# jwliao1209/DiffMusic

Hardware: AMD Instinct MI355X
Metric: denoising steps/sec (10 s clip, 200-step DPS) (higher is better)
Workload: dtype f16; 1 GPU; MusicLDM + DPS music_inpainting, 10 s @16 kHz, 200-step schedule, batch 8 per GPU (BASELINE.json configs[1]); global_batch=8, clips_per_gpu=8, lanes=1, parallelism=clip-sharded x1 (RCCL world size 1, no per-step collective), finite=True, nan_steps=0, settle_steps=10, cached_reference_transform=True, launched_by=single process

## Files before the change

diffmusic_amd/_lib.py:

```python
import ctypes as C
import os

_HERE = os.path.dirname(os.path.abspath(__file__))
LIB_PATH = os.environ.get("DMX_LIB_PATH") or os.path.join(_HERE, "lib", "libdiffmusic_hip.so")
MAX_STAGES = 8


class HifiGanConfig(C.Structure):
    _fields_ = [("model_in_dim", C.c_int), ("upsample_initial_channel", C.c_int), ("num_upsamples", C.c_int),
                ("upsample_rates", C.c_int * MAX_STAGES), ("upsample_kernel_sizes", C.c_int * MAX_STAGES),
                ("num_kernels", C.c_int), ("resblock_kernel_sizes", C.c_int * MAX_STAGES),
                ("num_dilations", C.c_int), ("resblock_dilation_sizes", C.c_int * (MAX_STAGES * MAX_STAGES)),
                ("leaky_relu_slope", C.c_float)]


class VaeConfig(C.Structure):
    _fields_ = [("latent_channels", C.c_int), ("out_channels", C.c_int), ("num_blocks", C.c_int),
                ("block_out_channels", C.c_int * MAX_STAGES), ("layers_per_block", C.c_int),
                ("norm_num_groups", C.c_int), ("eps", C.c_float)]


class UNetConfig(C.Structure):
    _fields_ = [("in_channels", C.c_int), ("out_channels", C.c_int), ("num_blocks", C.c_int),
                ("block_out_channels", C.c_int * MAX_STAGES), ("layers_per_block", C.c_int),
# ... 46 lines not shown
    "dmx_model_param_numel": (C.c_size_t, [C.c_void_p, C.c_int]),
    "dmx_model_param_ndim": (C.c_int, [C.c_void_p, C.c_int]),
    "dmx_model_param_dim": (C.c_int, [C.c_void_p, C.c_int, C.c_int]),
    "dmx_model_load_param": (C.c_int, [C.c_void_p, C.c_char_p, C.c_void_p, C.c_size_t]),
    "dmx_model_finalize": (C.c_int, [C.c_void_p, C.c_void_p]),
    "dmx_hifigan_out_len": (C.c_int, [C.c_void_p, C.c_int]),
    "dmx_hifigan_workspace_bytes": (C.c_size_t, [C.c_void_p, C.c_int, C.c_int]),
    "dmx_hifigan_fwd": (C.c_int, [C.c_void_p, C.c_void_p, C.c_void_p, C.c_int, C.c_int, C.c_void_p, C.c_size_t, C.c_void_p]),
    "dmx_hifigan_bwd": (C.c_int, [C.c_void_p, C.c_void_p, C.c_void_p, C.c_void_p]),
    "dmx_hifigan_fwd_dead": (C.c_int, [C.c_void_p, C.c_void_p, C.c_void_p, C.c_int, C.c_int, C.c_int, C.c_int, C.c_void_p, C.c_size_t,
                                       C.c_void_p]),
    "dmx_hifigan_dead_plan": (C.c_int, [C.c_void_p, C.POINTER(C.c_int), C.POINTER(C.c_int), C.POINTER(C.c_int), C.POINTER(C.c_int), C.c_int]),
    "dmx_conv_dead_rows": (C.c_int, [C.c_int] * 9 + [C.POINTER(C.c_int), C.POINTER(C.c_int)]),
    "dmx_vae_workspace_bytes": (C.c_size_t, [C.c_void_p, C.c_int, C.c_int, C.c_int]),
    "dmx_vae_decode_fwd": (C.c_int, [C.c_void_p, C.c_void_p, C.c_float, C.c_void_p, C.c_void_p, C.c_int, C.c_int, C.c_int,
                                     C.c_int, C.c_void_p, C.c_size_t, C.c_void_p]),
    "dmx_vae_decode_bwd": (C.c_int, [C.c_void_p, C.c_void_p, C.c_float, C.c_void_p, C.c_void_p]),
    "dmx_vae_encoder_create": (C.c_void_p, [C.POINTER(VaeConfig)]),
    "dmx_vae_encoder_workspace_bytes": (C.c_size_t, [C.c_void_p, C.c_int, C.c_int, C.c_int]),
    "dmx_vae_encode_fwd": (C.c_int, [C.c_void_p, C.c_void_p, C.c_float, C.c_void_p, C.c_int, C.c_int, C.c_int, C.c_void_p, C.c_size_t,
                                     C.c_void_p]),
    "dmx_latent_init": (C.c_int, [C.c_void_p] * 6 + [C.c_int] * 3 + [C.c_float] * 3 + [C.c_void_p]),
    "dmx_conv2d_raw": (C.c_int, [C.c_void_p] * 4 + [C.c_int] * 9 + [C.c_void_p]),
    "dmx_unet_workspace_bytes": (C.c_size_t, [C.c_void_p, C.c_int, C.c_int, C.c_int]),
    "dmx_unet_fwd": (C.c_int, [C.c_void_p, C.c_void_p, C.c_void_p, C.c_void_p, C.c_void_p, C.c_int, C.c_int, C.c_int,
                               C.c_void_p, C.c_size_t, C.c_void_p]),
    "dmx_unet_fwd_ctx": (C.c_int, [C.c_void_p] * 5 + [C.c_int, C.c_void_p, C.c_int, C.c_void_p, C.c_void_p, C.c_int, C.c_int, C.c_int,
                                   C.c_void_p, C.c_size_t, C.c_void_p]),
    "dmx_unet_workspace_bytes_ctx": (C.c_size_t, [C.c_void_p, C.c_int, C.c_int, C.c_int, C.c_int, C.c_int]),
    "dmx_htsat_create": (C.c_void_p, [C.POINTER(HtsatConfig)]),
    "dmx_htsat_feature_dims": (C.c_int, [C.c_void_p, C.POINTER(C.c_int), C.POINTER(C.c_int)]),
    "dmx_htsat_workspace_bytes": (C.c_size_t, [C.c_void_p, C.c_int, C.c_int]),
    "dmx_htsat_fwd": (C.c_int, [C.c_void_p, C.c_void_p, C.c_int, C.c_int, C.c_void_p, C.c_int, C.c_void_p, C.c_size_t, C.c_void_p]),
    "dmx_htsat_bwd": (C.c_int, [C.c_void_p, C.c_void_p, C.c_void_p, C.c_void_p, C.c_void_p]),
    "dmx_htsat_tape_raw": (C.c_size_t, [C.c_void_p, C.c_int, C.c_int, C.c_int, C.c_void_p, C.c_size_t, C.c_void_p]),
    "dmx_htsat_ln_rows_fwd_raw": (C.c_int, [C.c_void_p] * 4 + [C.c_longlong] + [C.c_int] * 4 + [C.c_float, C.c_int, C.c_void_p]),
    "dmx_htsat_ln_rows_bwd_raw": (C.c_int, [C.c_void_p] * 5 + [C.c_longlong] + [C.c_int] * 4 + [C.c_float, C.c_int, C.c_void_p]),
    "dmx_htsat_gelu_fwd_raw": (C.c_int, [C.c_void_p, C.c_void_p, C.c_longlong, C.c_void_p]),
    "dmx_htsat_gelu_bwd_raw": (C.c_int, [C.c_void_p, C.c_void_p, C.c_void_p, C.c_longlong, C.c_void_p]),
    "dmx_htsat_win_attn_fwd_raw": (C.c_int, [C.c_void_p] * 3 + [C.c_int] * 6 + [C.c_void_p]),
    "dmx_htsat_win_attn_bwd_raw": (C.c_int, [C.c_void_p] * 4 + [C.c_int] * 6 + [C.c_void_p]),
    "dmx_htsat_embed_fwd_raw": (C.c_int, [C.c_void_p, C.c_void_p, C.c_int, C.c_int, C.c_void_p, C.c_void_p]),
    "dmx_htsat_embed_bwd_raw": (C.c_int, [C.c_void_p, C.c_void_p, C.c_int, C.c_int] + [C.c_void_p] * 5),
    "dmx_gram_fwd": (C.c_int, [C.c_void_p, C.c_void_p, C.c_int, C.c_int, C.c_int, C.c_void_p]),
    "dmx_gram_bwd": (C.c_int, [C.c_void_p, C.c_void_p, C.c_void_p, C.c_int, C.c_int, C.c_int, C.c_void_p]),
    "dmx_gemm_raw": (C.c_int, [C.c_void_p, C.c_size_t, C.c_void_p]),
# ... 167 lines not shown
```

diffmusic_amd/csrc/capi.hip:

```cpp
#include "conv_pair.h"
#include "models.h"

#define M_IMPL(m) ((m) ? (m)->impl : nullptr)
#define ST(s) ((hipStream_t)(s))

extern "C" {

int dmx_abi_version(void) { return DMX_ABI_VERSION; }
int dmx_act_dtype(void) { return DMX_ACT_DTYPE; }

dmx_model* dmx_hifigan_create(const dmx_hifigan_config* cfg) {
  if (!cfg || cfg->num_upsamples > DMX_MAX_STAGES || cfg->num_kernels > DMX_MAX_STAGES || cfg->num_dilations > DMX_MAX_STAGES) {
    dmx_set_error("bad hifigan config");
    return nullptr;
  }
  return new dmx_model{dmx_make_hifigan(cfg)};
}
dmx_model* dmx_vae_decoder_create(const dmx_vae_config* cfg) {
  if (!cfg || cfg->num_blocks > DMX_MAX_STAGES) { dmx_set_error("bad vae config"); return nullptr; }
  Model* m = dmx_make_vae(cfg);
  return m ? new dmx_model{m} : nullptr;
}
dmx_model* dmx_unet_create(const dmx_unet_config* cfg) {
  if (!cfg || cfg->num_blocks > DMX_MAX_STAGES) { dmx_set_error("bad unet config"); return nullptr; }
// ... 74 lines not shown
dmx_model* dmx_vae_encoder_create(const dmx_vae_config* cfg) {
  if (!cfg || cfg->num_blocks > DMX_MAX_STAGES) { dmx_set_error("bad vae config"); return nullptr; }
  Model* m = dmx_make_vae_encoder(cfg);
  return m ? new dmx_model{m} : nullptr;
}
size_t dmx_vae_encoder_workspace_bytes(dmx_model* m, int batch, int frames, int bins) {
  if (!m || !m->impl || m->impl->kind != DMX_MODEL_VAE_ENC) return 0;
  return dmx_vae_enc_ws_impl(m->impl, batch, frames, bins);
}
int dmx_vae_encode_fwd(dmx_model* m, const float* mel, float log_floor, float* moments, int batch, int frames, int bins, void* ws,
                       size_t ws_bytes, void* stream) {
  int rc = check(m, DMX_MODEL_VAE_ENC);
  if (rc) return rc;
  if (!ws) { dmx_set_error("null workspace"); return DMX_ERR_WORKSPACE; }
  return dmx_vae_enc_fwd_impl(m->impl, mel, log_floor, moments, batch, frames, bins, ws, ws_bytes, ST(stream));
}
int dmx_latent_init(const float* moments, float* mean, float* logvar, float* x, const float* eps, const float* noise, int batch,
                    int latent_channels, int hw, float sqrt_abar, float scaling_factor, float sqrt_1m_abar, void* stream) {
  return dmx_latent_init_impl(moments, mean, logvar, x, eps, noise, batch, latent_channels, hw, sqrt_abar, scaling_factor, sqrt_1m_abar, ST(stream));
}
int dmx_conv2d_raw(const float* w_host, const float* b_host, const void* x, void* y, int B, int Hi, int Wi, int Ci, int Co, int k, int stride,
                   int pad_lo, int pad_hi, void* stream) {
  return dmx_conv2d_raw_impl(w_host, b_host, (const act_t*)x, (act_t*)y, B, Hi, Wi, Ci, Co, k, stride, pad_lo, pad_hi, ST(stream));
}

dmx_model* dmx_htsat_create(const dmx_htsat_config* cfg) {
  Model* impl = dmx_make_htsat(cfg);
  if (!impl) return nullptr;
  return new dmx_model{impl};
}
int dmx_htsat_feature_dims(dmx_model* m, int* tokens, int* channels) {
  if (!m || !m->impl || m->impl->kind != DMX_MODEL_HTSAT) { dmx_set_error("wrong model handle"); return DMX_ERR_STATE; }
  dmx_htsat_dims_impl(m->impl, tokens, channels);
  return DMX_OK;
}
size_t dmx_htsat_workspace_bytes(dmx_model* m, int batch, int frames) {
  if (!m || !m->impl || m->impl->kind != DMX_MODEL_HTSAT) return 0;
  return dmx_htsat_ws_impl(m->impl, batch, frames);
}
int dmx_htsat_fwd(dmx_model* m, const float* mel, int batch, int frames, float* feat, int keep_state, void* ws, size_t ws_bytes, void* stream) {
  int rc = check(m, DMX_MODEL_HTSAT);
  if (rc) return rc;
  if (!ws) { dmx_set_error("null workspace"); return DMX_ERR_WORKSPACE; }
  return dmx_htsat_fwd_impl(m->impl, mel, batch, frames, feat, keep_state, ws, ws_bytes, ST(stream));
}
int dmx_htsat_bwd(dmx_model* m, const float* dfeat, const float* scale, float* dmel, void* stream) {
// ... 259 lines not shown
```

diffmusic_amd/csrc/kernels.h:

```cpp
#pragma once
#include "dmx_common.h"

#define DMX_GN_MAX_CHUNKS 512

size_t dmx_gn_scratch_floats(int B, int C, int G);
struct GnRegion {
  float* part = nullptr;
  int tm = 0, P = 0, nq = 0;
  int qoff = 0, cq = 0;
};
struct GnParts { int n = 0; GnRegion r[8]; };
size_t dmx_gn_part_floats(int B, int P, int N);
int dmx_groupnorm_fwd(const act_t* x, act_t* y, const float* gamma, const float* beta, float* stats, float* scale,
                      float* shift, float* partial, int B, int P, int C, int G, float eps, int silu, hipStream_t st,
                      const GnParts* parts = nullptr);
int dmx_groupnorm_bwd(const act_t* x, const act_t* dy, const act_t* add, act_t* dx, const float* stats,
                      const float* scale, const float* shift, float* k0, float* k1, float* partial, int B, int P, int C,
                      int G, int silu, hipStream_t st, const GnParts* parts = nullptr);
int dmx_layernorm_fwd(const act_t* x, act_t* y, const float* gamma, const float* beta, int rows, int C, float eps,
                      hipStream_t st);
int dmx_softmax_fwd(const float* S, act_t* P, const float* colbias, long long rows, int N, long long lds, long long ldp,
                    int rows_per_bias, hipStream_t st);
int dmx_softmax_act(const act_t* S, act_t* P, const float* colbias, long long rows, int N, long long ldp, int rows_per_bias,
                    hipStream_t st);
// ... 5 lines not shown
int dmx_transpose(const act_t* in, act_t* out, int R, int C, long long ldi, long long ldo, int Z, int Zi, long long sIo,
                  long long sIi, long long sOo, long long sOi, hipStream_t st);
int dmx_concat2(const act_t* a, const act_t* b, act_t* dst, long long rows, int Ca, int Cb, hipStream_t st);
int dmx_copy_channels(const act_t* src, act_t* dst, long long rows, int C, int lds, int ldd, int soff, int doff,
                      hipStream_t st);
int dmx_axpby(const act_t* x, const act_t* y0, act_t* y, float a, float b, long long n, hipStream_t st);
int dmx_nchw_f32_to_nhwc_bf16(const float* x, act_t* y, int B, int C, int HW, int Cp, float scale, hipStream_t st);
int dmx_nhwc_bf16_to_nchw_f32(const act_t* x, float* y, int B, int C, int HW, int Cp, float scale, hipStream_t st);
int dmx_f32_to_bf16(const float* x, act_t* y, long long n, float scale, hipStream_t st);
int dmx_bf16_to_f32(const act_t* x, float* y, long long n, float scale, hipStream_t st);
int dmx_extract_col(const act_t* x, float* y, long long rows, int ld, int col, hipStream_t st);
int dmx_gather_col_f32(const float* x, float* y, long long rows, int ld, int col, hipStream_t st);
int dmx_tanh_bwd_pad8(const float* dwav, const float* wav8, act_t* gz, long long rows, hipStream_t st);
int dmx_gather_col_f32_dead(const float* x, float* y, long long rows, int ld, int col, int T, int s0, int s1, hipStream_t st);
int dmx_tanh_bwd_pad8_dead(const float* dwav, const float* wav8, act_t* gz, long long rows, int T, int s0, int s1, hipStream_t st);
int dmx_scatter_col_pad8(const float* v, act_t* y, long long rows, float scale, hipStream_t st);
int dmx_gather_col_f32_to_act(const float* x, act_t* y, long long rows, int ld, int col, hipStream_t st);
int dmx_pad_col8_act(const act_t* v, act_t* y, long long rows, hipStream_t st);
int dmx_timestep_embed(const float* t, act_t* y, int B, int dim, hipStream_t st);

bool dmx_flash_attn_ok(int dh, int C);
int dmx_flash_attn_fwd(const act_t* q, const act_t* k, const act_t* v, act_t* o, const float* colbias, int B, int Nq, int Nk,
                       int C, int heads, float scale, hipStream_t st, int ldq = 0, int ldk = 0, int ldv = 0, int* qt_out = nullptr);

int dmx_stft_tables(float* table, float* tableT, int n_fft, int bins, int Npad, int Kpad, int hann, hipStream_t st);
int dmx_stft_fwd(const float* wav, long long wav_stride, const float* table, float* X, int B, int L, int T, int n_fft, int hop, int Npad,
                 hipStream_t st);
int dmx_stft_bwd_frames(const float* Y, const float* tableT, float* dframe, int M, int n_fft, int Kpad, hipStream_t st);
int dmx_mel_fwd(const float* X, const float* fb, float* mel_lin, float* mel_out, int rows, int ldx, int bins, int n_mels, int power2,
                int to_db, float lo, float hi, hipStream_t st);
int dmx_mel_bwd(const float* X, const float* fb, const float* mel_lin, const float* dmel, float* Y, int rows, int ldx, int ldy, int bins,
                int n_mels, int power2, int to_db, float lo, float hi, hipStream_t st);
int dmx_stft_mag(const float* X, float* mag, int B, int T, int bins, int ldx, hipStream_t st);
int dmx_stft_mag_bwd(const float* X, const float* dmag, float* Y, int B, int T, int bins, int ldx, int ldy, hipStream_t st);
int dmx_overlap_add(const float* dframe, float* dwav, long long out_stride, int B, int T, int L, int n_fft, int hop, int accumulate,
                    hipStream_t st);
int dmx_l2_loss_grad(const float* ref, const float* pred, float* loss, float* dpred, int B, long long n, long long ref_stride, float gscale,
                     hipStream_t st);
int dmx_mask_mul(const float* x, long long xs, const float* mask, float* y, long long ys, int B, int L, int Ly, hipStream_t st);
int dmx_melscale(const float* mag, const float* fb, float* mel, int B, int T, int bins, int n_mels, float lo, float hi, hipStream_t st);
int dmx_absmax_normalize(float* x, float* inv_scale, int B, long long n, float target, hipStream_t st);

struct DmxStftMelTables {
  const float2* tw;
  const float* win;
  const int *klo, *klen; const float* fbc; int kmax;
// ... 40 lines not shown
```

diffmusic_amd/csrc/layers.h:

```cpp
#pragma once
#include <string>
#include <vector>
#include <map>
#include <cstdio>
#include <cstring>
#include "dmx_common.h"
#include "kernels.h"

void dmx_set_error(const char* fmt, ...);

inline int pad8(int c) { return (c + 7) & ~7; }

struct Arena {
  char* base = nullptr;
  size_t cap = 0, off = 0, peak = 0;
  bool overflow = false;
  void reset(void* b, size_t c) { base = (char*)b; cap = c; off = 0; overflow = false; }
  void* raw(size_t bytes) {
    bytes = align_up(bytes, 256);
    if (off + bytes > cap) { overflow = true; off += bytes; if (off > peak) peak = off; return base; }
    void* p = base + off;
    off += bytes;
    if (off > peak) peak = off;
    return p;
// ... 72 lines not shown
ConvLayer make_linear(ParamStore& ps, const std::string& prefix, int Ci, int Co, bool bias, bool need_bwd);
int pack_layer(ParamStore& ps, ConvLayer& L, hipStream_t st);
int pack_linear_stack(ParamStore& ps, ConvLayer& dst, const ConvLayer* const* src, int n, hipStream_t st);

int conv_out_len(const ConvLayer& L, int Ti);
int conv_fwd_1d(const ConvLayer& L, const act_t* in, void* out, int B, int Ti, const Epi& e, hipStream_t st);
int conv_bwd_1d(const ConvLayer& L, const act_t* dout, void* din, int B, int Ti, const Epi& e, hipStream_t st);
int conv_fwd_1d_desc(const ConvLayer& L, const act_t* in, void* out, int B, int Ti, const Epi& e, GemmDesc& d);
int conv_bwd_1d_desc(const ConvLayer& L, const act_t* dout, void* din, int B, int Ti, const Epi& e, GemmDesc& d);
struct PairDead;
int conv_pair_run(const GemmDesc& a, const GemmDesc& b, hipStream_t st, const PairDead* dead = nullptr);
int conv_fwd_2d(const ConvLayer& L, const act_t* in, void* out, int B, int Hi, int Wi, const Epi& e, hipStream_t st, int* gn_rows = nullptr);
int pack_layer_up2x(ParamStore& ps, ConvLayer& L, hipStream_t st);
int conv_up2x_fwd(const ConvLayer& L, const act_t* in, void* out, int B, int Hi, int Wi, const Epi& e, hipStream_t st,
                  float* const* gn_buf = nullptr, int* gn_rows = nullptr);
int conv_up2x_bwd(const ConvLayer& L, const act_t* dout, void* din, int B, int Hi, int Wi, const Epi& e, hipStream_t st);
int conv_bwd_2d(const ConvLayer& L, const act_t* dout, void* din, int B, int Hi, int Wi, const Epi& e, hipStream_t st, int* gn_rows = nullptr);
struct GemmBatch { int Z = 1, Zi = 1; long long sAo = 0, sAi = 0, sBo = 0, sBi = 0, sCo = 0, sCi = 0; };
int gemm_nt(const act_t* A, int lda, const act_t* Bm, int ldb, void* C, int ldc, int M, int N, int K, const Epi& e,
            const GemmBatch& gb, hipStream_t st);
int linear_fwd(const ConvLayer& L, const act_t* in, int lda, void* out, int ldc, long long rows, const Epi& e, hipStream_t st);
int linear_bwd(const ConvLayer& L, const act_t* dout, int lda, void* din, int ldc, long long rows, const Epi& e, hipStream_t st);

struct GroupNormLayer {
  int C = 0, G = 32, g_id = -1, b_id = -1;
  float eps = 1e-5f;
};
GroupNormLayer make_gn(ParamStore& ps, const std::string& prefix, int C, int G, float eps);
struct GnSave { float* stats = nullptr; float* scale = nullptr; float* shift = nullptr; };
```

diffmusic_amd/csrc/layers.hip:

```cpp
#include "layers.h"
#include "conv_pair.h"
#include <cstdarg>

static thread_local char g_err[512] = "";
void dmx_set_error(const char* fmt, ...) {
  va_list ap;
  va_start(ap, fmt);
  vsnprintf(g_err, sizeof(g_err), fmt, ap);
  va_end(ap);
}
extern "C" const char* dmx_last_error() { return g_err; }

int ParamStore::add(const std::string& name, std::vector<int> shape) {
  Param p;
  p.name = name;
  p.shape = shape;
  p.numel = 1;
  for (int s : shape) p.numel *= (size_t)s;
  p.dev = (float*)dalloc(p.numel * sizeof(float));
  index[name] = (int)params.size();
  params.push_back(p);
  return (int)params.size() - 1;
}
void* ParamStore::dalloc(size_t bytes) {
// ... 275 lines not shown
  return rc;
}

static void init_desc(GemmDesc& d, const Epi& e) {
  memset(&d, 0, sizeof(d));
  d.Z = 1; d.Zi = 1;
  d.sy = d.sx = 1; d.osy = d.osx = 1;
  d.alpha = e.alpha; d.act_slope = e.act_slope; d.mask_slope = e.mask_slope; d.resid_inv_slope = e.resid_inv_slope;
  d.flags = e.flags;
  d.R = e.R; d.X = e.X; d.C2 = e.C2; d.rowbias = e.rowbias; d.ldrb = e.ldrb;
  d.XB = e.XB; d.B2 = e.B2;
  d.rowstats_out = e.rowstats_out; d.rowstats_in = e.rowstats_in; d.nslots = e.nslots;
  d.gn_part = e.gn_part;
  if (e.gn_part) d.flags |= e.gnb_x ? EPI_GNBWD : EPI_GNSTATS;
  d.gnb_x = e.gnb_x; d.gnb_scale = e.gnb_scale; d.gnb_shift = e.gnb_shift; d.gnb_silu = e.gnb_silu;
  d.gnb_stats = e.gnb_stats; d.gnb_cpg = e.gnb_cpg;
}
static void set_out(GemmDesc& d, void* C, int Ho, int Wo, int ldc) {
  d.C = C; d.Ho = Ho; d.Wo = Wo; d.ldc = d.ldr = d.ldx = d.ldc2 = ldc;
  d.ldxb = d.ldb2 = ldc >> 3;
  d.gnb_ldx = ldc;
}

int conv_out_len(const ConvLayer& L, int Ti) {
  if (L.transposed) return (Ti - 1) * L.stride - 2 * L.pad_w + L.kw;
  return (Ti + 2 * L.pad_w - L.dil * (L.kw - 1) - 1) / L.stride + 1;
}

static void fwd_1d_common(GemmDesc& d, const ConvLayer& L, const act_t* in, void* out, int Ti, int To, const Epi& e) {
  init_desc(d, e);
  if (L.has_bias) { d.bias = L.bias; d.flags |= EPI_BIAS; }
  d.A = in; d.Hi = 1; d.Wi = Ti; d.Ci = L.Cip; d.lda = L.Cip;
  d.N = L.Cop;
  set_out(d, out, 1, To, L.Cop);
}
int conv_fwd_1d_desc(const ConvLayer& L, const act_t* in, void* out, int B, int Ti, const Epi& e, GemmDesc& d) {
  if (L.transposed) return DMX_ERR_SHAPE;
  const int To = conv_out_len(L, Ti);
  fwd_1d_common(d, L, in, out, Ti, To, e);
  d.W = L.wf[0]; d.ntaps = L.kw; d.K = L.kw * L.Cip; d.ldw = d.K;
  d.Hq = 1; d.Wq = To; d.sx = L.stride; d.M = B * To;
  for (int t = 0; t < L.kw; ++t) { d.tdy[t] = 0; d.tdx[t] = (signed char)(t * L.dil - L.pad_w); }
  return DMX_OK;
}

int conv_fwd_1d(const ConvLayer& L, const act_t* in, void* out, int B, int Ti, const Epi& e, hipStream_t st) {
  const int To = conv_out_len(L, Ti);
  GemmDesc d;
  if (!L.transposed) {
    const int rc = conv_fwd_1d_desc(L, in, out, B, Ti, e, d);
    return rc != DMX_OK ? rc : dmx_gemm_launch(d, st);
  }
  fwd_1d_common(d, L, in, out, Ti, To, e);
  const int s = L.stride, p = L.pad_w;
  for (int r = 0; r < s; ++r) {
    GemmDesc q = d;
    const int nt = (int)L.wf_taps[r].size();
    const int base = (r + p) / s;
    q.W = L.wf[r]; q.ntaps = nt; q.K = nt * L.Cip; q.ldw = q.K;
    q.Hq = 1; q.Wq = cdiv(To - r, s); q.M = B * q.Wq;
    q.osx = s; q.oox = r;
    for (int i = 0; i < nt; ++i) { q.tdy[i] = 0; q.tdx[i] = (signed char)(base - i); }
    if (q.Wq <= 0) continue;
    const int rc = dmx_gemm_launch(q, st);
    if (rc != DMX_OK) return rc;
  }
  return DMX_OK;
}

int conv_bwd_1d_desc(const ConvLayer& L, const act_t* dout, void* din, int B, int Ti, const Epi& e, GemmDesc& d) {
  if (!L.wb) { dmx_set_error("layer has no dgrad weights"); return DMX_ERR_STATE; }
  const int To = conv_out_len(L, Ti);
  init_desc(d, e);
  d.A = dout; d.Hi = 1; d.Wi = To; d.Ci = L.Cop; d.lda = L.Cop;
  d.W = L.wb; d.ntaps = L.kw; d.K = L.kw * L.Cop; d.ldw = d.K;
  d.N = L.Cip;
  d.Hq = 1; d.Wq = Ti; d.M = B * Ti;
  set_out(d, din, 1, Ti, L.Cip);
  if (!L.transposed) {
    if (L.stride != 1) return DMX_ERR_SHAPE;
    for (int t = 0; t < L.kw; ++t) { d.tdy[t] = 0; d.tdx[t] = (signed char)(L.pad_w - t * L.dil); }
  } else {
    d.sx = L.stride;
    for (int t = 0; t < L.kw; ++t) { d.tdy[t] = 0; d.tdx[t] = (signed char)(t - L.pad_w); }
  }
  return DMX_OK;
}
int conv_bwd_1d(const ConvLayer& L, const act_t* dout, void* din, int B, int Ti, const Epi& e, hipStream_t st) {
  GemmDesc d;
  const int rc = conv_bwd_1d_desc(L, dout, din, B, Ti, e, d);
  return rc != DMX_OK ? rc : dmx_gemm_launch(d, st);
}

int conv_pair_run(const GemmDesc& a, const GemmDesc& b, hipStream_t st, const PairDead* dead) {
  if (dmx_conv_pair_eligible(&a, b)) return dmx_conv_pair_launch(&a, b, st, dead);
  if (dead) { dmx_set_error("conv_pair_run: dead rows need the fused pair kernel"); return DMX_ERR_SHAPE; }
  const int rc = dmx_gemm_launch(a, st);
  return rc != DMX_OK ? rc : dmx_gemm_launch(b, st);
}

int conv_fwd_2d(const ConvLayer& L, const act_t* in, void* out, int B, int Hi, int Wi, const Epi& e, hipStream_t st, int* gn_rows) {
  const int Ho = (Hi + L.pad_h + L.pad_h_hi - L.kh) / L.stride + 1, Wo = (Wi + L.pad_w + L.pad_w_hi - L.kw) / L.stride + 1;
  GemmDesc d;
  init_desc(d, e);
  if (L.has_bias) { d.bias = L.bias; d.flags |= EPI_BIAS; }
  d.A = in; d.Hi = Hi; d.Wi = Wi; d.Ci = L.Cip; d.lda = L.Cip;
  d.W = L.wf[0]; d.ntaps = L.kh * L.kw; d.K = d.ntaps * L.Cip; d.ldw = d.K;
  d.N = L.Cop; d.Hq = Ho; d.Wq = Wo; d.sy = d.sx = L.stride; d.M = B * Ho * Wo;
  set_out(d, out, Ho, Wo, L.Cop);
  for (int ky = 0; ky < L.kh; ++ky)
    for (int kx = 0; kx < L.kw; ++kx) {
      d.tdy[ky * L.kw + kx] = (signed char)(ky - L.pad_h);
      d.tdx[ky * L.kw + kx] = (signed char)(kx - L.pad_w);
    }
  return dmx_gemm_launch(d, st, gn_rows);
}

int conv_up2x_fwd(const ConvLayer& L, const act_t* in, void* out, int B, int Hi, int Wi, const Epi& e, hipStream_t st,
                  float* const* gn_buf, int* gn_rows) {
  if (L.wup.size() != 4) { dmx_set_error("layer has no upsample-folded weights"); return DMX_ERR_STATE; }
  for (int py = 0; py < 2; ++py)
    for (int px = 0; px < 2; ++px) {
      GemmDesc d;
      Epi ep = e;
      if (gn_buf) ep.gn_part = gn_buf[py * 2 + px];
      init_desc(d, ep);
      if (L.has_bias) { d.bias = L.bias; d.flags |= EPI_BIAS; }
      d.A = in; d.Hi = Hi; d.Wi = Wi; d.Ci = L.Cip; d.lda = L.Cip;
      d.W = L.wup[py * 2 + px]; d.ntaps = 4; d.K = 4 * L.Cip; d.ldw = d.K;
      d.N = L.Cop; d.Hq = Hi; d.Wq = Wi; d.M = B * Hi * Wi;
      set_out(d, out, 2 * Hi, 2 * Wi, L.Cop);
      d.osy = d.osx = 2; d.ooy = py; d.oox = px;
      for (int ty = 0; ty < 2; ++ty)
        for (int tx = 0; tx < 2; ++tx) {
          d.tdy[ty * 2 + tx] = (signed char)up2x_delta(py, ty);
          d.tdx[ty * 2 + tx] = (signed char)up2x_delta(px, tx);
        }
// ... 16 lines not shown
      const int t = (py * 2 + ty) * 4 + (px * 2 + tx);
      d.tdy[t] = (signed char)(py - 2 * up2x_delta(py, ty));
      d.tdx[t] = (signed char)(px - 2 * up2x_delta(px, tx));
    }
  return dmx_gemm_launch(d, st);
}

int conv_bwd_2d(const ConvLayer& L, const act_t* dout, void* din, int B, int Hi, int Wi, const Epi& e, hipStream_t st, int* gn_rows) {
  if (!L.wb) { dmx_set_error("layer has no dgrad weights"); return DMX_ERR_STATE; }
  if (L.stride != 1) return DMX_ERR_SHAPE;
  if (L.pad_h_hi != L.pad_h || L.pad_w_hi != L.pad_w) { dmx_set_error("conv dgrad of an asymmetrically padded layer is not built"); return DMX_ERR_SHAPE; }
  const int Ho = Hi + 2 * L.pad_h - L.kh + 1, Wo = Wi + 2 * L.pad_w - L.kw + 1;
  GemmDesc d;
  init_desc(d, e);
  d.A = dout; d.Hi = Ho; d.Wi = Wo; d.Ci = L.Cop; d.lda = L.Cop;
  d.W = L.wb; d.ntaps = L.kh * L.kw; d.K = d.ntaps * L.Cop; d.ldw = d.K;
  d.N = L.Cip; d.Hq = Hi; d.Wq = Wi; d.M = B * Hi * Wi;
  set_out(d, din, Hi, Wi, L.Cip);
  for (int ky = 0; ky < L.kh; ++ky)
    for (int kx = 0; kx < L.kw; ++kx) {
      d.tdy[ky * L.kw + kx] = (signed char)(L.pad_h - ky);
      d.tdx[ky * L.kw + kx] = (signed char)(L.pad_w - kx);
    }
  return dmx_gemm_launch(d, st, gn_rows);
}

int gemm_nt(const act_t* A, int lda, const act_t* Bm, int ldb, void* C, int ldc, int M, int N, int K, const Epi& e,
            const GemmBatch& gb, hipStream_t st) {
  GemmDesc d;
  init_desc(d, e);
  d.A = A; d.Hi = 1; d.Wi = M; d.Ci = K; d.lda = lda;
  d.W = Bm; d.ntaps = 1; d.K = K; d.ldw = ldb;
  d.N = N; d.Hq = 1; d.Wq = M; d.M = M;
  set_out(d, C, 1, M, ldc);
  d.Z = gb.Z; d.Zi = gb.Zi;
  d.sAo = gb.sAo; d.sAi = gb.sAi; d.sWo = gb.sBo; d.sWi = gb.sBi; d.sCo = gb.sCo; d.sCi = gb.sCi;
  return dmx_gemm_launch(d, st);
}

int linear_fwd(const ConvLayer& L, const act_t* in, int lda, void* out, int ldc, long long rows, const Epi& e, hipStream_t st) {
  Epi ee = e;
  GemmDesc d;
  init_desc(d, ee);
  if (L.has_bias) { d.bias = L.bias; d.flags |= EPI_BIAS; }
  d.A = in; d.Hi = 1; d.Wi = (int)rows; d.Ci = L.Cip; d.lda = lda;
  d.W = L.wf[0]; d.ntaps = 1; d.K = L.Cip; d.ldw = L.Cip;
  d.N = L.Cop; d.Hq = 1; d.Wq = (int)rows; d.M = (int)rows;
  set_out(d, out, 1, (int)rows, ldc);
  if (L.geglu) d.flags |= EPI_GEGLU;
  if (L.colsum) {
    if (!e.rowstats_in || e.nslots * 32 != L.Cip) { dmx_set_error("LayerNorm-folded layer needs the row statistics of its input"); return DMX_ERR_STATE; }
    d.flags |= EPI_LNFOLD; d.colsum = L.colsum; d.ln_eps = L.ln_eps;
    d.flags &= ~EPI_BIAS;
  }
  return dmx_gemm_launch(d, st);
}
int linear_bwd(const ConvLayer& L, const act_t* dout, int lda, void* din, int ldc, long long rows, const Epi& e, hipStream_t st) {
  if (!L.wb) { dmx_set_error("layer has no dgrad weights"); return DMX_ERR_STATE; }
  GemmDesc d;
  init_desc(d, e);
  d.A = dout; d.Hi = 1; d.Wi = (int)rows; d.Ci = L.Cop; d.lda = lda;
  d.W = L.wb; d.ntaps = 1; d.K = L.Cop; d.ldw = L.Cop;
  d.N = L.Cip; d.Hq = 1; d.Wq = (int)rows; d.M = (int)rows;
  set_out(d, din, 1, (int)rows, ldc);
  return dmx_gemm_launch(d, st);
}
```

include/diffmusic_hip.h:

```cpp
#ifndef DIFFMUSIC_HIP_H
#define DIFFMUSIC_HIP_H
#include <stddef.h>
#include <stdint.h>

#ifdef __cplusplus
extern "C" {
#endif

#define DMX_ABI_VERSION 4
#define DMX_MAX_STAGES 8

typedef struct dmx_model dmx_model;

typedef struct dmx_hifigan_config {
  int model_in_dim;
  int upsample_initial_channel;
  int num_upsamples;
  int upsample_rates[DMX_MAX_STAGES];
  int upsample_kernel_sizes[DMX_MAX_STAGES];
  int num_kernels;
  int resblock_kernel_sizes[DMX_MAX_STAGES];
  int num_dilations;
  int resblock_dilation_sizes[DMX_MAX_STAGES * DMX_MAX_STAGES];
  float leaky_relu_slope;
// ... 226 lines not shown
                          int ldk, int ldv, int C, int heads, float scale, int* qt_out, void* stream);
int dmx_softmax_raw(const float* S, void* P, const float* colbias, long long rows, int N, long long lds, long long ldp, int rows_per_bias,
                    void* stream);
int dmx_softmax_act_raw(const void* S, void* P, const float* colbias, long long rows, int N, long long ldp, int rows_per_bias, void* stream);
int dmx_transpose_raw(const void* in, void* out, int R, int C, long long ldi, long long ldo, int Z, int Zi, long long sIo, long long sIi,
                      long long sOo, long long sOi, void* stream);
int dmx_rowdot_raw(const void* a, const void* b, float* out, long long rows, int C, long long lda, long long ldb, void* stream);
int dmx_layernorm_raw(const void* x, void* y, const float* gamma, const float* beta, int rows, int C, float eps, void* stream);
int dmx_geglu_raw(const void* x, void* y, long long rows, int I, void* stream);
int dmx_gemm_splitk_workspace(void* ws, size_t bytes);
int dmx_conv_pair_raw(const void* desc_a, const void* desc_b, size_t desc_bytes, void* stream);
int dmx_conv_pair_dead_raw(const void* desc_a, const void* desc_b, size_t desc_bytes, const int* dead, int* skipped, int* total, void* stream);
int dmx_conv_pair_group_raw(int n, const void* descs_a, const void* descs_b, size_t desc_bytes, void* stream);
int dmx_conv_pair_group_dead_raw(int n, const void* descs_a, const void* descs_b, size_t desc_bytes, const int* dead, void* stream);
size_t dmx_groupnorm_scratch_floats(int B, int C, int G);
int dmx_groupnorm_raw(const void* x, void* y, const float* gamma, const float* beta, float* stats, float* scale, float* shift,
                      float* partial, int B, int P, int C, int G, float eps, int silu, void* stream);
size_t dmx_groupnorm_part_floats(int B, int P, int N);
int dmx_groupnorm_parts_raw(const void* x, void* y, const float* gamma, const float* beta, float* stats, float* scale, float* shift,
                            int B, int P, int C, int G, float eps, int silu, int nreg, float* const* part, const int* geom, void* stream);
int dmx_gemm_last_tile_rows_raw(void);
int dmx_conv2d_raw(const float* w_host, const float* b_host, const void* x, void* y, int B, int Hi, int Wi, int Ci, int Co, int k, int stride,
                   int pad_lo, int pad_hi, void* stream);
int dmx_groupnorm_bwd_raw(const void* x, const void* dy, const void* add, void* dx, const float* stats, const float* scale, const float* shift,
                          float* k0, float* k1, float* partial, int B, int P, int C, int G, int silu, int nreg, float* const* part,
                          const int* geom, void* stream);
int dmx_htsat_ln_rows_fwd_raw(const void* x, void* y, const float* gamma, const float* beta, long long rows, int C, int merge, int H, int W,
                              float eps, int out_fp32, void* stream);
int dmx_htsat_ln_rows_bwd_raw(const void* x, const void* dy, const void* add, void* dx, const float* gamma, long long rows, int C, int merge,
                              int H, int W, float eps, int dy_fp32, void* stream);
int dmx_htsat_gelu_fwd_raw(const void* u, void* y, long long n8, void* stream);
int dmx_htsat_gelu_bwd_raw(const void* u, const void* dy, void* du, long long n8, void* stream);
int dmx_htsat_win_attn_fwd_raw(const void* qkv, void* out, const float* bias_table, int B, int H, int W, int C, int heads, int shift,
                               void* stream);
int dmx_htsat_win_attn_bwd_raw(const void* qkv, const void* dout, void* dqkv, const float* bias_table, int B, int H, int W, int C, int heads,
                               int shift, void* stream);
int dmx_htsat_embed_fwd_raw(dmx_model* m, const float* mel, int batch, int frames, void* tokens, void* stream);
int dmx_htsat_embed_bwd_raw(dmx_model* m, const float* mel, int batch, int frames, const void* dtok, const float* scale, float* dimg,
                            float* dmel, void* stream);

#ifdef __cplusplus
}
#endif
#endif
```

Baseline: 27.47 steps/s (weak scaling: one step advances a batch of 8 clips on one GPU; value = K / wall x 1 GPU(s)).

## Add narrow-output conv kernels for head convolutions with few output channels

Adds dedicated HIP kernels for convolutions whose output is at most 8 channels (padded to 8), such as the HiFi-GAN output conv and VAE conv_out. The forward kernel stages an input halo slab in LDS and uses packed fdot2 dot products, with optional split-K reduction. A separate dgrad kernel handles the single-output 1D backward with the mask epilogue. These replace the general GEMM path, whose tiles are mostly wasted when N is 8. It also adds a test hook for the new path and a DMX_NO_NARROW env switch. The risk is extra code paths with their own edge cases, including numerics that differ from the GEMM path.

Result: no change. 27.56 steps/s (weak scaling: one step advances a batch of 8 clips on one GPU; value = K / wall x 1 GPU(s)) (median of 6 runs) (+0.3%).

```diff
diff --git a/diffmusic_amd/_lib.py b/diffmusic_amd/_lib.py
--- a/diffmusic_amd/_lib.py
+++ b/diffmusic_amd/_lib.py
@@ -92,6 +92,7 @@
                                      C.c_void_p]),
     "dmx_latent_init": (C.c_int, [C.c_void_p] * 6 + [C.c_int] * 3 + [C.c_float] * 3 + [C.c_void_p]),
     "dmx_conv2d_raw": (C.c_int, [C.c_void_p] * 4 + [C.c_int] * 9 + [C.c_void_p]),
+    "dmx_head_conv_raw": (C.c_int, [C.c_int] + [C.c_void_p] * 5 + [C.c_int] * 7 + [C.c_float, C.c_float, C.POINTER(C.c_int), C.c_void_p]),
     "dmx_unet_workspace_bytes": (C.c_size_t, [C.c_void_p, C.c_int, C.c_int, C.c_int]),
     "dmx_unet_fwd": (C.c_int, [C.c_void_p, C.c_void_p, C.c_void_p, C.c_void_p, C.c_void_p, C.c_int, C.c_int, C.c_int,
                                C.c_void_p, C.c_size_t, C.c_void_p]),
diff --git a/diffmusic_amd/csrc/capi.hip b/diffmusic_amd/csrc/capi.hip
--- a/diffmusic_amd/csrc/capi.hip
+++ b/diffmusic_amd/csrc/capi.hip
@@ -120,6 +120,12 @@
 int dmx_conv2d_raw(const float* w_host, const float* b_host, const void* x, void* y, int B, int Hi, int Wi, int Ci, int Co, int k, int stride,
                    int pad_lo, int pad_hi, void* stream) {
   return dmx_conv2d_raw_impl(w_host, b_host, (const act_t*)x, (act_t*)y, B, Hi, Wi, Ci, Co, k, stride, pad_lo, pad_hi, ST(stream));
+}
+
+int dmx_head_conv_raw(int kind, const float* w_host, const float* b_host, const void* x, const void* mask, void* y, int B, int H, int W, int Ci,
+                      int Co, int k, int flags, float alpha, float mask_slope, int* route, void* stream) {
+  return dmx_head_conv_raw_impl(kind, w_host, b_host, (const act_t*)x, (const act_t*)mask, y, B, H, W, Ci, Co, k, flags, alpha, mask_slope, route,
+                                ST(stream));
 }
 
 dmx_model* dmx_htsat_create(const dmx_htsat_config* cfg) {
diff --git a/diffmusic_amd/csrc/kernels.h b/diffmusic_amd/csrc/kernels.h
--- a/diffmusic_amd/csrc/kernels.h
+++ b/diffmusic_amd/csrc/kernels.h
@@ -51,6 +51,22 @@
 bool dmx_flash_attn_ok(int dh, int C);
 int dmx_flash_attn_fwd(const act_t* q, const act_t* k, const act_t* v, act_t* o, const float* colbias, int B, int Nq, int Nk,
                        int C, int heads, float scale, hipStream_t st, int ldq = 0, int ldk = 0, int ldv = 0, int* qt_out = nullptr);
+
+struct NarrowConvDesc {
+  const act_t* in = nullptr;
+  const act_t* w = nullptr;
+  const float* bias = nullptr;
+  void* out = nullptr;
+  int B = 0, H = 1, W = 0, Cip = 0, nout = 0, ntaps = 0;
+  signed char tdy[DMX_MAX_TAPS] = {}, tdx[DMX_MAX_TAPS] = {};
+  float alpha = 1.f;
+  int flags = 0;
+};
+bool dmx_narrow_conv_ok(const NarrowConvDesc& d);
+int dmx_narrow_conv_launch(const NarrowConvDesc& d, hipStream_t st);
+bool dmx_narrow_dgrad_ok(int Cip, int k, int dil, int flags);
+int dmx_narrow_dgrad_launch(const act_t* gz, const act_t* wb, const act_t* X, act_t* din, int B, int T, int Cip, int k, int dil, int pad,
+                            float alpha, float mask_slope, int flags, hipStream_t st);
 
 int dmx_stft_tables(float* table, float* tableT, int n_fft, int bins, int Npad, int Kpad, int hann, hipStream_t st);
 int dmx_stft_fwd(const float* wav, long long wav_stride, const float* table, float* X, int B, int L, int T, int n_fft, int hop, int Npad,
diff --git a/diffmusic_amd/csrc/layers.h b/diffmusic_amd/csrc/layers.h
--- a/diffmusic_amd/csrc/layers.h
+++ b/diffmusic_amd/csrc/layers.h
@@ -118,6 +118,10 @@
 int linear_fwd(const ConvLayer& L, const act_t* in, int lda, void* out, int ldc, long long rows, const Epi& e, hipStream_t st);
 int linear_bwd(const ConvLayer& L, const act_t* dout, int lda, void* din, int ldc, long long rows, const Epi& e, hipStream_t st);
 
+int narrow_last_route();
+int dmx_head_conv_raw_impl(int kind, const float* w_host, const float* b_host, const act_t* x, const act_t* mask, void* y, int B, int H, int W,
+                           int Ci, int Co, int k, int flags, float alpha, float mask_slope, int* route, hipStream_t st);
+
 struct GroupNormLayer {
   int C = 0, G = 32, g_id = -1, b_id = -1;
   float eps = 1e-5f;
diff --git a/diffmusic_amd/csrc/layers.hip b/diffmusic_amd/csrc/layers.hip
--- a/diffmusic_amd/csrc/layers.hip
+++ b/diffmusic_amd/csrc/layers.hip
@@ -321,6 +321,23 @@
   d.gnb_ldx = ldc;
 }
 
+static thread_local int g_narrow_route = 0;
+int narrow_last_route() { return g_narrow_route; }
+static bool narrow_on() { return getenv("DMX_NO_NARROW") == nullptr; }
+static bool narrow_plain_map(const GemmDesc& d) {
+  return d.sy == 1 && d.sx == 1 && d.osy == 1 && d.osx == 1 && d.ooy == 0 && d.oox == 0 && d.Ho == d.Hi && d.Wo == d.Wi && d.Hq == d.Hi &&
+         d.Wq == d.Wi && d.Z == 1 && d.lda == d.Ci && d.ldw == d.K && !d.gn_part && !d.tile_cfg;
+}
+static bool narrow_fwd_take(const GemmDesc& d, int nreal, NarrowConvDesc& n) {
+  if (!narrow_on() || nreal < 1 || nreal > 8 || d.N != 8 || d.ldc != 8 || !narrow_plain_map(d)) return false;
+  n.in = d.A; n.w = d.W; n.bias = d.bias; n.out = d.C;
+  n.H = d.Hi; n.W = d.Wi; n.Cip = d.Ci; n.nout = nreal == 1 ? 1 : 8; n.ntaps = d.ntaps;
+  n.B = d.M / (d.Hi * d.Wi);
+  memcpy(n.tdy, d.tdy, sizeof(n.tdy)); memcpy(n.tdx, d.tdx, sizeof(n.tdx));
+  n.alpha = d.alpha; n.flags = d.flags;
+  return dmx_narrow_conv_ok(n);
+}
+
 int conv_out_len(const ConvLayer& L, int Ti) {
   if (L.transposed) return (Ti - 1) * L.stride - 2 * L.pad_w + L.kw;
   return (Ti + 2 * L.pad_w - L.dil * (L.kw - 1) - 1) / L.stride + 1;
@@ -348,8 +365,12 @@
   GemmDesc d;
   if (!L.transposed) {
     const int rc = conv_fwd_1d_desc(L, in, out, B, Ti, e, d);
-    return rc != DMX_OK ? rc : dmx_gemm_launch(d, st);
-  }
+    if (rc != DMX_OK) return rc;
+    NarrowConvDesc n;
+    g_narrow_route = narrow_fwd_take(d, L.Co, n) ? 1 : 0;
+    return g_narrow_route ? dmx_narrow_conv_launch(n, st) : dmx_gemm_launch(d, st);
+  }
+  g_narrow_route = 0;
   fwd_1d_common(d, L, in, out, Ti, To, e);
   const int s = L.stride, p = L.pad_w;
   for (int r = 0; r < s; ++r) {
@@ -388,7 +409,11 @@
 int conv_bwd_1d(const ConvLayer& L, const act_t* dout, void* din, int B, int Ti, const Epi& e, hipStream_t st) {
   GemmDesc d;
   const int rc = conv_bwd_1d_desc(L, dout, din, B, Ti, e, d);
-  return rc != DMX_OK ? rc : dmx_gemm_launch(d, st);
+  if (rc != DMX_OK) return rc;
+  g_narrow_route = narrow_on() && !L.transposed && L.Co == 1 && L.Cop == 8 && narrow_plain_map(d) && d.ldc == L.Cip && d.ldx == L.Cip &&
+                   d.alpha == e.alpha && dmx_narrow_dgrad_ok(L.Cip, L.kw, L.dil, d.flags) ? 1 : 0;
+  if (g_narrow_route) return dmx_narrow_dgrad_launch(dout, L.wb, e.X, (act_t*)din, B, Ti, L.Cip, L.kw, L.dil, L.pad_w, e.alpha, e.mask_slope, d.flags, st);
+  return dmx_gemm_launch(d, st);
 }
 
 int conv_pair_run(const GemmDesc& a, const GemmDesc& b, hipStream_t st, const PairDead* dead) {
@@ -412,6 +437,9 @@
       d.tdy[ky * L.kw + kx] = (signed char)(ky - L.pad_h);
       d.tdx[ky * L.kw + kx] = (signed char)(kx - L.pad_w);
     }
+  NarrowConvDesc n;
+  g_narrow_route = narrow_fwd_take(d, L.Co, n) ? 1 : 0;
+  if (g_narrow_route) { if (gn_rows) *gn_rows = 0; return dmx_narrow_conv_launch(n, st); }
   return dmx_gemm_launch(d, st, gn_rows);
 }
 
@@ -474,6 +502,9 @@
       d.tdy[ky * L.kw + kx] = (signed char)(L.pad_h - ky);
       d.tdx[ky * L.kw + kx] = (signed char)(L.pad_w - kx);
     }
+  NarrowConvDesc n;
+  g_narrow_route = narrow_fwd_take(d, L.Ci, n) ? 1 : 0;
+  if (g_narrow_route) { if (gn_rows) *gn_rows = 0; return dmx_narrow_conv_launch(n, st); }
   return dmx_gemm_launch(d, st, gn_rows);
 }
 
@@ -517,3 +548,30 @@
   set_out(d, din, 1, (int)rows, ldc);
   return dmx_gemm_launch(d, st);
 }
+
+int dmx_head_conv_raw_impl(int kind, const float* w_host, const float* b_host, const act_t* x, const act_t* mask, void* y, int B, int H, int W,
+                           int Ci, int Co, int k, int flags, float alpha, float mask_slope, int* route, hipStream_t st) {
+  const bool two_d = kind == 1 || kind == 3, bwd = kind >= 2;
+  if (kind < 0 || kind > 3 || B < 1 || H < 1 || W < 1 || Ci < 1 || Co < 1 || k < 1 || !(k & 1) || (two_d ? k * k : k) > DMX_MAX_TAPS || (!two_d && H != 1)) {
+    dmx_set_error("head_conv_raw: bad geometry");
+    return DMX_ERR_SHAPE;
+  }
+  if (flags & ~(bwd ? EPI_MASK : (EPI_TANH | EPI_F32OUT))) { dmx_set_error("head_conv_raw: flag not offered by this hook"); return DMX_ERR_SHAPE; }
+  ParamStore ps;
+  ConvLayer L = two_d ? make_conv2d(ps, "conv", Ci, Co, k, 1, k / 2, bwd) : make_conv1d(ps, "conv", Ci, Co, k, 1, k / 2, bwd);
+  int rc = ps.load("conv.weight", w_host, (size_t)Co * Ci * (two_d ? k * k : k));
+  if (rc == DMX_OK) rc = ps.load("conv.bias", b_host, (size_t)Co);
+  if (rc == DMX_OK) rc = pack_layer(ps, L, st);
+  Epi e;
+  e.flags = flags; e.alpha = alpha; e.mask_slope = mask_slope; e.X = mask;
+  if (rc == DMX_OK) {
+    if (kind == 0) rc = conv_fwd_1d(L, x, y, B, W, e, st);
+    else if (kind == 1) rc = conv_fwd_2d(L, x, y, B, H, W, e, st);
+    else if (kind == 2) rc = conv_bwd_1d(L, x, y, B, W, e, st);
+    else rc = conv_bwd_2d(L, x, y, B, H, W, e, st);
+  }
+  if (route) *route = narrow_last_route();
+  (void)hipStreamSynchronize(st);
+  ps.free_all();
+  return rc;
+}
diff --git a/diffmusic_amd/csrc/narrow_conv.hip b/diffmusic_amd/csrc/narrow_conv.hip
--- /dev/null
+++ b/diffmusic_amd/csrc/narrow_conv.hip
@@ -0,0 +1,272 @@
+#include "dmx_common.h"
+#include "kernels.h"
+#include "conv_pair.h"
+
+namespace {
+
+constexpr int NC_THREADS = 256;
+constexpr int NC_CG = 32;
+constexpr int NC_LB = 8;
+
+__device__ __forceinline__ float nc_dot8(const uint4& x, const uint4& w, float acc) {
+#ifndef DMX_BF16
+  typedef _Float16 nc_h2 __attribute__((ext_vector_type(2)));
+  acc = __builtin_amdgcn_fdot2(__builtin_bit_cast(nc_h2, x.x), __builtin_bit_cast(nc_h2, w.x), acc, false);
+  acc = __builtin_amdgcn_fdot2(__builtin_bit_cast(nc_h2, x.y), __builtin_bit_cast(nc_h2, w.y), acc, false);
+  acc = __builtin_amdgcn_fdot2(__builtin_bit_cast(nc_h2, x.z), __builtin_bit_cast(nc_h2, w.z), acc, false);
+  acc = __builtin_amdgcn_fdot2(__builtin_bit_cast(nc_h2, x.w), __builtin_bit_cast(nc_h2, w.w), acc, false);
+#else
+  acc = __builtin_fmaf(alo(x.x), alo(w.x), acc); acc = __builtin_fmaf(ahi(x.x), ahi(w.x), acc);
+  acc = __builtin_fmaf(alo(x.y), alo(w.y), acc); acc = __builtin_fmaf(ahi(x.y), ahi(w.y), acc);
+  acc = __builtin_fmaf(alo(x.z), alo(w.z), acc); acc = __builtin_fmaf(ahi(x.z), ahi(w.z), acc);
+  acc = __builtin_fmaf(alo(x.w), alo(w.w), acc); acc = __builtin_fmaf(ahi(x.w), ahi(w.w), acc);
+#endif
+  return acc;
+}
+
+struct NarrowGeom {
+  int H, W, P;
+  int Cip, ntaps, ldw;
+  int lo, span;
+  float alpha;
+  int flags;
+  int toff[DMX_MAX_TAPS];
+  int tdyx[DMX_MAX_TAPS];
+};
+
+template <int NO, int KS>
+__global__ __launch_bounds__(NC_THREADS) void narrow_conv_kernel(const act_t* __restrict__ in, const act_t* __restrict__ w,
+                                                                const float* __restrict__ bias, void* __restrict__ out, NarrowGeom g) {
+  constexpr int R = NC_THREADS / KS;
+  constexpr int CPP = KS * (NC_CG / 8);
+  constexpr int PITCH = CPP * 16 + 16;
+  extern __shared__ __attribute__((aligned(16))) char nc_slab[];
+  const int tid = threadIdx.x;
+  const int r = tid % R, kq = KS == 1 ? 0 : __builtin_amdgcn_readfirstlane(tid / R);
+  const int p0 = blockIdx.x * R, p = p0 + r;
+  const int s0 = p0 - g.lo;
+  const int npix = R + g.span;
+  const act_t* img = in + (long long)blockIdx.y * g.P * g.Cip;
+  unsigned okmask = 0;
+  {
+    const int y = p / g.W, x = p - y * g.W;
+    for (int t = 0; t < g.ntaps; ++t) {
+      const int yy = y + (g.tdyx[t] >> 16), xx = x + (short)(g.tdyx[t] & 0xffff);
+      if (p < g.P && yy >= 0 && yy < g.H && xx >= 0 && xx < g.W) okmask |= 1u << t;
+    }
+  }
+  float acc[NO];
+#pragma unroll
+  for (int n = 0; n < NO; ++n) acc[n] = 0.f;
+  for (int c0 = 0; c0 < g.Cip; c0 += KS * NC_CG) {
+    const int nch = min(KS * NC_CG, g.Cip - c0) >> 3;
+    __syncthreads();
+    for (int i0 = tid; i0 < npix * CPP; i0 += NC_LB * NC_THREADS) {
+      uint4 v[NC_LB];
+#pragma unroll
+      for (int u = 0; u < NC_LB; ++u) {
+        const int i = i0 + u * NC_THREADS;
+        const int sp = i / CPP, ch = i - sp * CPP;
+        const int fp = s0 + sp;
+        v[u] = make_uint4(0u, 0u, 0u, 0u);
+        if (i < npix * CPP && ch < nch && fp >= 0 && fp < g.P) v[u] = *reinterpret_cast<const uint4*>(img + (long long)fp * g.Cip + c0 + ch * 8);
+      }
+#pragma unroll
+      for (int u = 0; u < NC_LB; ++u) {
+        const int i = i0 + u * NC_THREADS;
+        const int sp = i / CPP, ch = i - sp * CPP;
+        if (i < npix * CPP) *reinterpret_cast<uint4*>(nc_slab + sp * PITCH + ch * 16) = v[u];
+      }
+    }
+    __syncthreads();
+    const int cb = kq * (NC_CG / 8);
+    for (int t = 0; t < g.ntaps; ++t) {
+      const int off = g.toff[t];
+      const bool ok = (okmask >> t) & 1u;
+      const char* src = nc_slab + (r + off) * PITCH + cb * 16;
+      const act_t* wt = w + (long long)t * g.Cip + c0 + cb * 8;
+#pragma unroll
+      for (int ch = 0; ch < NC_CG / 8; ++ch) {
+        if (cb + ch < nch) {
+          uint4 xv = *reinterpret_cast<const uint4*>(src + ch * 16);
+          if (!ok) xv = make_uint4(0u, 0u, 0u, 0u);
+#pragma unroll
+          for (int n = 0; n < NO; ++n) {
+            const uint4 wv = *reinterpret_cast<const uint4*>(wt + (long long)n * g.ldw + ch * 8);
+            acc[n] = nc_dot8(xv, wv, acc[n]);
+          }
+        }
+      }
+    }
+  }
+  if constexpr (KS > 1) {
+    float* red = reinterpret_cast<float*>(nc_slab);
+    __syncthreads();
+#pragma unroll
+    for (int n = 0; n < NO; ++n) red[(kq * R + r) * NO + n] = acc[n];
+    __syncthreads();
+    if (kq != 0) return;
+#pragma unroll
+    for (int n = 0; n < NO; ++n) {
+      float s = red[r * NO + n];
+#pragma unroll
+      for (int q = 1; q < KS; ++q) s += red[(q * R + r) * NO + n];
+      acc[n] = s;
+    }
+  }
+  if (p >= g.P) return;
+  float v[8];
+#pragma unroll
+  for (int n = 0; n < 8; ++n) v[n] = n < NO ? acc[n] : 0.f;
+  if (g.flags & EPI_BIAS) {
+#pragma unroll
+    for (int n = 0; n < 8; ++n) v[n] += bias[n];
+  }
+  const float al = g.alpha;
+#pragma unroll
+  for (int n = 0; n < 8; ++n) v[n] *= al;
+  if (g.flags & EPI_TANH) {
+#pragma unroll
+    for (int n = 0; n < 8; ++n) v[n] = n < NO ? tanhf(v[n]) : v[n];
+  }
+  const long long orow = (long long)blockIdx.y * g.P + p;
+  if (g.flags & EPI_F32OUT) {
+    float4* o = reinterpret_cast<float4*>(reinterpret_cast<float*>(out) + orow * 8);
+    o[0] = make_float4(v[0], v[1], v[2], v[3]);
+    o[1] = make_float4(v[4], v[5], v[6], v[7]);
+  } else {
+    *reinterpret_cast<uint4*>(reinterpret_cast<act_t*>(out) + orow * 8) =
+        make_uint4(pack2a(v[0], v[1]), pack2a(v[2], v[3]), pack2a(v[4], v[5]), pack2a(v[6], v[7]));
+  }
+}
+
+constexpr int ND_ROWS = 256;
+template <int NCHK>
+__global__ __launch_bounds__(NC_THREADS) void narrow_dgrad_kernel(const act_t* __restrict__ gz, const act_t* __restrict__ wb,
+                                                                 const act_t* __restrict__ X, act_t* __restrict__ din, int T, int k, int dil,
+                                                                 int pad, float alpha, float mask_slope, int flags) {
+  constexpr int Cip = NCHK * 8;
+  __shared__ float gl[ND_ROWS + DMX_MAX_TAPS * DMX_MAX_TAPS];
+  __shared__ __attribute__((aligned(16))) float wl[DMX_MAX_TAPS * Cip];
+  const int tid = threadIdx.x;
+  const int t0 = blockIdx.x * ND_ROWS;
+  const int span = (k - 1) * dil;
+  const int s0 = t0 + pad - span;
+  const long long clip = (long long)blockIdx.y * T;
+  for (int i = tid; i < ND_ROWS + span; i += NC_THREADS) {
+    const int ft = s0 + i;
+    float v = 0.f;
+    if (ft >= 0 && ft < T) v = alo(reinterpret_cast<const uint4*>(gz + (clip + ft) * 8)->x);
+    gl[i] = v;
+  }
+  for (int i = tid; i < k * Cip; i += NC_THREADS) {
+    const int j = i / Cip, c = i - j * Cip;
+    wl[i] = a2f(wb[((long long)c * k + j) * 8]);
+  }
+  __syncthreads();
+  const int chunk = tid % NCHK, rb = tid / NCHK;
+  constexpr int RSTEP = NC_THREADS / NCHK;
+  uint4 xm[NCHK];
+  if (flags & EPI_MASK) {
+#pragma unroll
+    for (int it = 0; it < NCHK; ++it) {
+      const int t = t0 + rb + it * RSTEP;
+      xm[it] = *reinterpret_cast<const uint4*>(X + (clip + (t < T ? t : 0)) * Cip + chunk * 8);
+    }
+  }
+#pragma unroll
+  for (int it = 0; it < NCHK; ++it) {
+    const int rr = rb + it * RSTEP, t = t0 + rr;
+    float v[8] = {0.f, 0.f, 0.f, 0.f, 0.f, 0.f, 0.f, 0.f};
+    for (int j = 0; j < k; ++j) {
+      const float gv = gl[rr + (k - 1 - j) * dil];
+      const float4 w0 = *reinterpret_cast<const float4*>(wl + j * Cip + chunk * 8);
+      const float4 w1 = *reinterpret_cast<const float4*>(wl + j * Cip + chunk * 8 + 4);
+      v[0] = __builtin_fmaf(gv, w0.x, v[0]); v[1] = __builtin_fmaf(gv, w0.y, v[1]);
+      v[2] = __builtin_fmaf(gv, w0.z, v[2]); v[3] = __builtin_fmaf(gv, w0.w, v[3]);
+      v[4] = __builtin_fmaf(gv, w1.x, v[4]); v[5] = __builtin_fmaf(gv, w1.y, v[5]);
+      v[6] = __builtin_fmaf(gv, w1.z, v[6]); v[7] = __builtin_fmaf(gv, w1.w, v[7]);
+    }
+    if (flags & EPI_MASK) {
+      const uint4 q = xm[it];
+      const float s = mask_slope;
+      v[0] *= alo(q.x) > 0.f ? 1.f : s; v[1] *= ahi(q.x) > 0.f ? 1.f : s;
+      v[2] *= alo(q.y) > 0.f ? 1.f : s; v[3] *= ahi(q.y) > 0.f ? 1.f : s;
+      v[4] *= alo(q.z) > 0.f ? 1.f : s; v[5] *= ahi(q.z) > 0.f ? 1.f : s;
+      v[6] *= alo(q.w) > 0.f ? 1.f : s; v[7] *= ahi(q.w) > 0.f ? 1.f : s;
+    }
+#pragma unroll
+    for (int e = 0; e < 8; ++e) v[e] *= alpha;
+    if (t < T)
+      *reinterpret_cast<uint4*>(din + (clip + t) * Cip + chunk * 8) =
+          make_uint4(pack2a(v[0], v[1]), pack2a(v[2], v[3]), pack2a(v[4], v[5]), pack2a(v[6], v[7]));
+  }
+}
+
+constexpr size_t NC_MAX_LDS = 64 * 1024;
+
+int nc_ks(int nout, int Cip) { return nout > 1 && Cip >= 4 * NC_CG ? 4 : 1; }
+size_t nc_lds_bytes(int ks, int span) { return (size_t)(NC_THREADS / ks + span) * (ks * (NC_CG / 8) * 16 + 16); }
+
+}
+
+bool dmx_narrow_conv_ok(const NarrowConvDesc& d) {
+  if (d.nout < 1 || d.nout > 8 || d.ntaps < 2 || d.ntaps > DMX_MAX_TAPS || d.Cip < 8 || (d.Cip & 7) || d.H < 1 || d.W < 1) return false;
+  if (d.flags & ~(EPI_BIAS | EPI_TANH | EPI_F32OUT)) return false;
+  if ((d.flags & EPI_BIAS) && !d.bias) return false;
+  int lo = 0, hi = 0;
+  for (int t = 0; t < d.ntaps; ++t) {
+    const int o = d.tdy[t] * d.W + d.tdx[t];
+    lo = o < lo ? o : lo; hi = o > hi ? o : hi;
+  }
+  return nc_lds_bytes(nc_ks(d.nout, d.Cip), hi - lo) <= NC_MAX_LDS;
+}
+
+int dmx_narrow_conv_launch(const NarrowConvDesc& d, hipStream_t st) {
+  if (!dmx_narrow_conv_ok(d) || d.B < 1 || d.B > 65535) { return DMX_ERR_SHAPE; }
+  NarrowGeom g;
+  memset(&g, 0, sizeof(g));
+  g.H = d.H; g.W = d.W; g.P = d.H * d.W; g.Cip = d.Cip; g.ntaps = d.ntaps; g.ldw = d.ntaps * d.Cip;
+  g.alpha = d.alpha; g.flags = d.flags;
+  int lo = 0, hi = 0;
+  for (int t = 0; t < d.ntaps; ++t) {
+    g.tdyx[t] = (int)((unsigned)d.tdy[t] << 16 | ((unsigned)d.tdx[t] & 0xffffu));
+    const int o = d.tdy[t] * d.W + d.tdx[t];
+    lo = o < lo ? o : lo; hi = o > hi ? o : hi;
+  }
+  g.lo = -lo; g.span = hi - lo;
+  for (int t = 0; t < d.ntaps; ++t) g.toff[t] = d.tdy[t] * d.W + d.tdx[t] + g.lo;
+  const int ks = nc_ks(d.nout, d.Cip);
+  const size_t lds = nc_lds_bytes(ks, g.span);
+  const dim3 grid((unsigned)cdiv(g.P, NC_THREADS / ks), (unsigned)d.B);
+  const int rec = dmx_prof_open(st);
+  if (d.nout == 1) hipLaunchKernelGGL((narrow_conv_kernel<1, 1>), grid, dim3(NC_THREADS), lds, st, d.in, d.w, d.bias, d.out, g);
+  else if (ks == 1) hipLaunchKernelGGL((narrow_conv_kernel<8, 1>), grid, dim3(NC_THREADS), lds, st, d.in, d.w, d.bias, d.out, g);
+  else hipLaunchKernelGGL((narrow_conv_kernel<8, 4>), grid, dim3(NC_THREADS), lds, st, d.in, d.w, d.bias, d.out, g);
+  const double M = (double)d.B * g.P, K = (double)d.ntaps * d.Cip;
+  dmx_prof_close(rec, st, 2.0 * M * 8 * K, 2.0 * M * d.Cip + 16.0 * K + M * 8 * ((d.flags & EPI_F32OUT) ? 4.0 : 2.0), (int)M, 8, (int)K, d.ntaps,
+                 d.flags, 40);
+  return hipGetLastError() == hipSuccess ? DMX_OK : DMX_ERR_LAUNCH;
+}
+
+bool dmx_narrow_dgrad_ok(int Cip, int k, int dil, int flags) {
+  if (Cip != 8 && Cip != 16 && Cip != 32 && Cip != 64) return false;
+  if (k < 2 || k > DMX_MAX_TAPS || dil < 1 || dil > DMX_MAX_TAPS) return false;
+  return !(flags & ~EPI_MASK);
+}
+
+int dmx_narrow_dgrad_launch(const act_t* gz, const act_t* wb, const act_t* X, act_t* din, int B, int T, int Cip, int k, int dil, int pad,
+                            float alpha, float mask_slope, int flags, hipStream_t st) {
+  if (!dmx_narrow_dgrad_ok(Cip, k, dil, flags) || B < 1 || B > 65535 || T < 1 || pad < 0 || ((flags & EPI_MASK) && !X)) return DMX_ERR_SHAPE;
+  const dim3 grid((unsigned)cdiv(T, ND_ROWS), (unsigned)B);
+  const int rec = dmx_prof_open(st);
+#define DMX_ND_LAUNCH(NCHK) hipLaunchKernelGGL((narrow_dgrad_kernel<NCHK>), grid, dim3(NC_THREADS), 0, st, gz, wb, X, din, T, k, dil, pad, alpha, mask_slope, flags)
+  if (Cip == 8) DMX_ND_LAUNCH(1);
+  else if (Cip == 16) DMX_ND_LAUNCH(2);
+  else if (Cip == 32) DMX_ND_LAUNCH(4);
+  else DMX_ND_LAUNCH(8);
+#undef DMX_ND_LAUNCH
+  const double M = (double)B * T;
+  dmx_prof_close(rec, st, 2.0 * M * Cip * k * 8, M * 16 + M * Cip * 2 * ((flags & EPI_MASK) ? 2.0 : 1.0), (int)M, Cip, k * 8, k, flags, 41);
+  return hipGetLastError() == hipSuccess ? DMX_OK : DMX_ERR_LAUNCH;
+}
diff --git a/include/diffmusic_hip.h b/include/diffmusic_hip.h
--- a/include/diffmusic_hip.h
+++ b/include/diffmusic_hip.h
@@ -272,6 +272,8 @@
 int dmx_gemm_last_tile_rows_raw(void);
 int dmx_conv2d_raw(const float* w_host, const float* b_host, const void* x, void* y, int B, int Hi, int Wi, int Ci, int Co, int k, int stride,
                    int pad_lo, int pad_hi, void* stream);
+int dmx_head_conv_raw(int kind, const float* w_host, const float* b_host, const void* x, const void* mask, void* y, int B, int H, int W, int Ci,
+                      int Co, int k, int flags, float alpha, float mask_slope, int* route, void* stream);
 int dmx_groupnorm_bwd_raw(const void* x, const void* dy, const void* add, void* dx, const float* stats, const float* scale, const float* shift,
                           float* k0, float* k1, float* partial, int B, int P, int C, int G, int silu, int nreg, float* const* part,
                           const int* geom, void* stream);
```
